# DCMMC/halo2-scaffold

Measured on AMD Instinct MI355X. Metric: create_proof() wall-clock + MSM G1-adds/s at k=20 standard_plonk, 1/2/4/8 GPU, higher is better.
Workload: dtype u32 (254-bit Montgomery integers as 9 x 29-bit limbs, 64-bit multiply-accumulate); 1 GPU; standard_plonk hot-path replay k=20: 11 MSM(2^20) + 6 iNTT(2^20) + 6 coset-NTT(2^21) + 1 coset-iNTT(2^21); k=20, scalar_distribution=uniform, msm_window_bits=17, msm_windows=15, msm_buckets=65536, parallelism=single-gpu, deployment=one process, one GPU, combine=none (single GPU)

## Files before the change

### halo2-scaffold_amd/csrc/f29.cuh

```cuda
#pragma once
#include <stdint.h>

#if defined(__HIPCC__)
#include <hip/hip_runtime.h>
#define H2_HD __host__ __device__ __forceinline__
#else
#define H2_HD inline
#endif

namespace h2 {

#include "f29_consts.inc"

constexpr uint32_t M29 = (1u << 29) - 1;

struct f29 {
  uint32_t v[9];
};

template <class F>
H2_HD f29 f29_const(const uint32_t (&c)[9]) {
  f29 r;
#pragma unroll
  for (int i = 0; i < 9; i++) r.v[i] = c[i];
  return r;
}
H2_HD f29 f29_zero() {
  f29 r;
#pragma unroll
  for (int i = 0; i < 9; i++) r.v[i] = 0;
  return r;
}
H2_HD bool f29_limbs_zero(const f29& a) {
  uint32_t o = 0;
#pragma unroll
  for (int i = 0; i < 9; i++) o |= a.v[i];
  return o == 0;
}

H2_HD f29 f29_unpack(const uint32_t w[8]) {
  f29 r;
#pragma unroll
  for (int i = 0; i < 9; i++) {
    const int bit = 29 * i, j = bit >> 5, s = bit & 31;
    uint32_t lo = w[j] >> s;
    if (s > 3 && j + 1 < 8) lo |= w[j + 1] << (32 - s);
    r.v[i] = (i < 8) ? (lo & M29) : lo;
  }
  return r;
}
H2_HD void f29_pack(const f29& a, uint32_t w[8]) {
#pragma unroll
  for (int j = 0; j < 8; j++) {
    const int bit = 32 * j, i = bit / 29, s = bit - 29 * i;
    uint32_t x = a.v[i] >> s;
    x |= a.v[i + 1] << (29 - s);
    if (29 - s + 29 < 32 && i + 2 < 9) x |= a.v[i + 2] << (58 - s);
    w[j] = x;
  }
}

H2_HD f29 f29_normalize(const f29& a) {
  f29 r;
  uint32_t c = 0;
#pragma unroll
  for (int i = 0; i < 8; i++) {
    uint32_t x = a.v[i] + c;
    r.v[i] = x & M29;
    c = x >> 29;
  }
  r.v[8] = a.v[8] + c;
  return r;
}

H2_HD f29 f29_add(const f29& a, const f29& b) {
  f29 r;
#pragma unroll
  for (int i = 0; i < 9; i++) r.v[i] = a.v[i] + b.v[i];
  return r;
}
H2_HD f29 f29_sub(const f29& a, const f29& b, const uint32_t (&K)[9]) {
  f29 r;
#pragma unroll
  for (int i = 0; i < 9; i++) r.v[i] = a.v[i] + K[i] - b.v[i];
  return r;
}
H2_HD f29 f29_dbl(const f29& a) {
  f29 r;
#pragma unroll
  for (int i = 0; i < 9; i++) r.v[i] = a.v[i] << 1;
  return r;
}

H2_HD void f29_mac_first(uint64_t& acc, uint32_t x, uint32_t y) {
#if defined(__HIP_DEVICE_COMPILE__)
  asm("v_mad_u64_u32 %0, vcc, %1, %2, %0" : "+v"(acc) : "v"(x), "v"(y) : "vcc");
#else
  acc += (uint64_t)x * y;
#endif
}

template <class F>
H2_HD f29 f29_mul(const f29& a, const f29& b) {
  uint32_t m[9];
  f29 t;
  uint64_t acc = 0;
#pragma unroll
  for (int k = 0; k < 9; k++) {
    f29_mac_first(acc, a.v[0], b.v[k]);
#pragma unroll
    for (int j = 1; j <= k; j++) acc += (uint64_t)a.v[j] * b.v[k - j];
#pragma unroll
    for (int j = 0; j < k; j++) acc += (uint64_t)m[j] * F::P[k - j];
    m[k] = ((uint32_t)acc * F::INV) & M29;
    acc += (uint64_t)m[k] * F::P[0];
    acc >>= 29;
  }
#pragma unroll
  for (int k = 9; k < 17; k++) {
    f29_mac_first(acc, a.v[k - 8], b.v[8]);
#pragma unroll
    for (int j = k - 7; j < 9; j++) acc += (uint64_t)a.v[j] * b.v[k - j];
#pragma unroll
    for (int j = k - 8; j < 9; j++) acc += (uint64_t)m[j] * F::P[k - j];
    t.v[k - 9] = (uint32_t)acc & M29;
    acc >>= 29;
  }
  t.v[8] = (uint32_t)acc;
  return t;
}
template <class F>
H2_HD f29 f29_mul2(const f29& a, const f29& b, const f29& c, const f29& d) {
  uint32_t m[9];
  f29 t;
  uint64_t acc = 0;
#pragma unroll
  for (int k = 0; k < 9; k++) {
    f29_mac_first(acc, a.v[0], b.v[k]);
#pragma unroll
    for (int j = 1; j <= k; j++) acc += (uint64_t)a.v[j] * b.v[k - j];
#pragma unroll
    for (int j = 0; j <= k; j++) acc += (uint64_t)c.v[j] * d.v[k - j];
#pragma unroll
    for (int j = 0; j < k; j++) acc += (uint64_t)m[j] * F::P[k - j];
    m[k] = ((uint32_t)acc * F::INV) & M29;
    acc += (uint64_t)m[k] * F::P[0];
    acc >>= 29;
  }
#pragma unroll
  for (int k = 9; k < 17; k++) {
    f29_mac_first(acc, a.v[k - 8], b.v[8]);
#pragma unroll
    for (int j = k - 7; j < 9; j++) acc += (uint64_t)a.v[j] * b.v[k - j];
#pragma unroll
    for (int j = k - 8; j < 9; j++) acc += (uint64_t)c.v[j] * d.v[k - j];
#pragma unroll
    for (int j = k - 8; j < 9; j++) acc += (uint64_t)m[j] * F::P[k - j];
    t.v[k - 9] = (uint32_t)acc & M29;
    acc >>= 29;
  }
  t.v[8] = (uint32_t)acc;
  return t;
}
template <class F>
H2_HD f29 f29_mul3(const f29& a, const f29& b, const f29& c, const f29& d, const f29& e, const f29& f) {
  uint32_t m[9];
  f29 t;
  uint64_t acc = 0;
#pragma unroll
  for (int k = 0; k < 9; k++) {
    f29_mac_first(acc, a.v[0], b.v[k]);
#pragma unroll
    for (int j = 1; j <= k; j++) acc += (uint64_t)a.v[j] * b.v[k - j];
#pragma unroll
    for (int j = 0; j <= k; j++) acc += (uint64_t)c.v[j] * d.v[k - j];
#pragma unroll
    for (int j = 0; j <= k; j++) acc += (uint64_t)e.v[j] * f.v[k - j];
#pragma unroll
    for (int j = 0; j < k; j++) acc += (uint64_t)m[j] * F::P[k - j];
    m[k] = ((uint32_t)acc * F::INV) & M29;
    acc += (uint64_t)m[k] * F::P[0];
    acc >>= 29;
  }
#pragma unroll
  for (int k = 9; k < 17; k++) {
    f29_mac_first(acc, a.v[k - 8], b.v[8]);
#pragma unroll
    for (int j = k - 7; j < 9; j++) acc += (uint64_t)a.v[j] * b.v[k - j];
#pragma unroll
    for (int j = k - 8; j < 9; j++) acc += (uint64_t)c.v[j] * d.v[k - j];
#pragma unroll
    for (int j = k - 8; j < 9; j++) acc += (uint64_t)e.v[j] * f.v[k - j];
#pragma unroll
    for (int j = k - 8; j < 9; j++) acc += (uint64_t)m[j] * F::P[k - j];
    t.v[k - 9] = (uint32_t)acc & M29;
    acc >>= 29;
  }
  t.v[8] = (uint32_t)acc;
  return t;
}
template <class F>
H2_HD f29 f29_sqr(const f29& a) {
  uint32_t m[9], a2[9];
#pragma unroll
  for (int i = 0; i < 9; i++) a2[i] = a.v[i] << 1;
  f29 t;
  uint64_t acc = 0;
#pragma unroll
  for (int k = 0; k < 9; k++) {
    if (k == 0) f29_mac_first(acc, a.v[0], a.v[0]);
    else f29_mac_first(acc, a.v[0], a2[k]);
#pragma unroll
    for (int j = 1; 2 * j < k; j++) acc += (uint64_t)a.v[j] * a2[k - j];
    if ((k & 1) == 0 && k > 0) acc += (uint64_t)a.v[k / 2] * a.v[k / 2];
#pragma unroll
    for (int j = 0; j < k; j++) acc += (uint64_t)m[j] * F::P[k - j];
    m[k] = ((uint32_t)acc * F::INV) & M29;
    acc += (uint64_t)m[k] * F::P[0];
    acc >>= 29;
  }
#pragma unroll
  for (int k = 9; k < 17; k++) {
    f29_mac_first(acc, m[k - 8], F::P[8]);
#pragma unroll
    for (int j = k - 8; 2 * j < k; j++) acc += (uint64_t)a.v[j] * a2[k - j];
    if ((k & 1) == 0) acc += (uint64_t)a.v[k / 2] * a.v[k / 2];
#pragma unroll
    for (int j = k - 7; j < 9; j++) acc += (uint64_t)m[j] * F::P[k - j];
    t.v[k - 9] = (uint32_t)acc & M29;
    acc >>= 29;
  }
  t.v[8] = (uint32_t)acc;
  return t;
}

template <class F>
H2_HD f29 f29_reduce_canonical(const f29& a) {
  f29 d;
  uint32_t borrow = 0;
#pragma unroll
  for (int i = 0; i < 9; i++) {
    uint32_t x = a.v[i] - F::P[i] - borrow;
    borrow = (x >> 31) & 1u;
    d.v[i] = (i < 8) ? (x & M29) : x;
  }
  f29 r;
#pragma unroll
  for (int i = 0; i < 9; i++) r.v[i] = borrow ? a.v[i] : d.v[i];
  return r;
}
template <class F>
H2_HD f29 f29_reduce_loose(const f29& a) {
  constexpr uint32_t M = (uint32_t)(((uint64_t)1 << 32) / (F::P[8] + 1));
  const uint32_t q = (uint32_t)(((uint64_t)a.v[8] * M) >> 32);
  f29 r;
  int64_t c = 0;
#pragma unroll
  for (int i = 0; i < 9; i++) {
    int64_t d = (int64_t)a.v[i] - (int64_t)((uint64_t)q * F::P[i]) + c;
    if (i < 8) {
      r.v[i] = (uint32_t)d & M29;
      c = d >> 29;
    } else {
      r.v[i] = (uint32_t)d;
    }
  }
  return f29_reduce_canonical<F>(f29_reduce_canonical<F>(r));
}

template <class F>
H2_HD bool f29_is_zero_mod(const f29& a) {
  if (a.v[0] != 0 && a.v[0] != F::P[0]) return false;
  uint32_t z = 0, e = 0;
#pragma unroll
  for (int i = 0; i < 9; i++) {
    z |= a.v[i];
    e |= a.v[i] ^ F::P[i];
  }
  return z == 0 || e == 0;
}

template <class F>
H2_HD f29 f29_inv(const f29& a) {
  f29 r = f29_const<F>(F::ONE);
  for (int i = 8; i >= 0; i--) {
    const uint32_t e = F::P[i] - (i == 0 ? 2u : 0u);
    const int top = (i == 8) ? 21 : 28;
    for (int b = top; b >= 0; b--) {
      r = f29_sqr<F>(r);
      if ((e >> b) & 1u) r = f29_mul<F>(r, a);
    }
  }
  return r;
}

template <class F>
H2_HD f29 f29_from_mont256(const uint32_t w[8]) {
  return f29_mul<F>(f29_unpack(w), f29_const<F>(F::TO261));
}
template <class F>
H2_HD void f29_to_mont256(const f29& a_norm, uint32_t w[8]) {
  f29 c = f29_reduce_canonical<F>(f29_mul<F>(a_norm, f29_const<F>(F::TO256)));
  f29_pack(c, w);
}

}
```

### halo2-scaffold_amd/csrc/f29_testops.cuh

```cuda
#pragma once
#include <stddef.h>

#include "g1_29.cuh"

namespace h2 {

template <class F>
H2_HD void f29t_mul_one(int mode, const uint32_t* a, const uint32_t* b, uint32_t* out) {
  if (mode == 0) {
    f29 x = f29_from_mont256<F>(a), y = f29_from_mont256<F>(b);
    f29_to_mont256<F>(f29_mul<F>(x, y), out);
  } else if (mode == 1) {
    f29 d = f29_unpack(a), w = f29_from_mont256<F>(b);
    f29 r = f29_reduce_canonical<F>(f29_mul<F>(d, w));
    f29_pack(r, out);
  } else if (mode == 2) {
    f29 x = f29_from_mont256<F>(a), y = f29_from_mont256<F>(b);
    f29 s = f29_normalize(f29_add(x, y));
    f29 d = f29_sub(x, y, F::K2);
    f29_to_mont256<F>(f29_mul<F>(d, s), out);
  } else if (mode == 4) {
    f29 x = f29_from_mont256<F>(a);
    f29_to_mont256<F>(f29_sqr<F>(x), out);
  } else if (mode == 5) {
    f29 x = f29_from_mont256<F>(a);
    f29_to_mont256<F>(f29_inv<F>(x), out);
  } else {
    f29 x = f29_unpack(a);
    f29_pack(x, out);
  }
}

H2_HD f29 f29t_load9(const uint32_t* p) {
  f29 x;
  for (int k = 0; k < 9; k++) x.v[k] = p[k];
  return x;
}
H2_HD void f29t_store9(const f29& x, uint32_t* p) {
  for (int k = 0; k < 9; k++) p[k] = x.v[k];
}

template <class F>
H2_HD void f29t_raw_one(int op, const uint32_t* a, const uint32_t* b, const uint32_t* c, const uint32_t* d, uint32_t* out) {
  f29 r;
  if (op == 0) r = f29_reduce_loose<F>(f29t_load9(a));
  else if (op == 1) r = f29_mul<F>(f29t_load9(a), f29t_load9(b));
  else if (op == 2) r = f29_sqr<F>(f29t_load9(a));
  else r = f29_mul2<F>(f29t_load9(a), f29t_load9(b), f29t_load9(c), f29t_load9(d));
  f29t_store9(r, out);
}
template <class F>
H2_HD void f29t_mul3_one(const uint32_t* ops, size_t n, size_t i, uint32_t* out) {
  f29 x[6];
  for (int q = 0; q < 6; q++) x[q] = f29t_load9(ops + ((size_t)q * n + i) * 9);
  f29t_store9(f29_mul3<F>(x[0], x[1], x[2], x[3], x[4], x[5]), out);
}

H2_HD bool f29t_table_point(const uint32_t* p, bool neg, f29& x2, f29& y2) {
  uint32_t any = 0;
  for (int k = 0; k < 16; k++) any |= p[k];
  if (any == 0) return false;
  uint32_t xw[8], yw[8];
  f29_pack(f29_reduce_canonical<Fq29>(f29_from_mont256<Fq29>(p)), xw);
  f29_pack(f29_reduce_canonical<Fq29>(f29_from_mont256<Fq29>(p + 8)), yw);
  x2 = f29_unpack(xw);
  y2 = f29_unpack(yw);
  if (neg) y2 = f29_sub(f29_zero(), y2, Fq29::K2);
  return true;
}

H2_HD void f29t_chain_one(const uint32_t* pts, const uint8_t* signs, size_t n, uint32_t* out_xyzz, int tree) {
  xyzz29 acc = xyzz29_identity();
  f29 x2, y2;
  if (!tree) {
    for (size_t i = 0; i < n; i++)
      if (f29t_table_point(pts + 16 * i, signs[i] != 0, x2, y2)) xyzz29_madd(acc, x2, y2);
  } else {
    xyzz29 groups[16];
    for (int g = 0; g < tree; g++) groups[g] = xyzz29_identity();
    for (size_t i = 0; i < n; i++)
      if (f29t_table_point(pts + 16 * i, signs[i] != 0, x2, y2)) xyzz29_madd(groups[i % tree], x2, y2);
    for (int stride = 1; stride < tree; stride *= 2)
      for (int g = 0; g + stride < tree; g += 2 * stride) xyzz29_add(groups[g], groups[g + stride]);
    acc = groups[0];
    if (tree == 16) {
      xyzz29 s2 = acc;
      xyzz29_add(s2, acc);
      xyzz29 d = xyzz29_dbl(acc);
      d.y = f29_normalize(f29_sub(f29_zero(), d.y, Fq29::K4));
      xyzz29_add(s2, d);
      xyzz29_add(s2, acc);
      acc = s2;
    }
  }
  if (xyzz29_is_identity(acc)) {
    for (int k = 0; k < 32; k++) out_xyzz[k] = 0;
    return;
  }
  f29_to_mont256<Fq29>(acc.x, out_xyzz);
  f29_to_mont256<Fq29>(acc.y, out_xyzz + 8);
  f29_to_mont256<Fq29>(acc.zz, out_xyzz + 16);
  f29_to_mont256<Fq29>(acc.zzz, out_xyzz + 24);
}

}
```

### halo2-scaffold_amd/csrc/g1_29.cuh

```cuda
#pragma once
#include "f29.cuh"

namespace h2 {

struct affine29 {
  f29 x, y;
};
struct xyzz29 {
  f29 x, y, zz, zzz;
};

H2_HD bool affine29_is_identity(const affine29& p) { return f29_limbs_zero(p.x) && f29_limbs_zero(p.y); }
H2_HD bool xyzz29_is_identity(const xyzz29& p) { return f29_limbs_zero(p.zz); }
H2_HD xyzz29 xyzz29_identity() {
  xyzz29 r;
  r.x = f29_zero(); r.y = f29_zero(); r.zz = f29_zero(); r.zzz = f29_zero();
  return r;
}

H2_HD xyzz29 xyzz29_dbl_affine(const f29& x, const f29& y_any) {
  using F = Fq29;
  xyzz29 r;
  f29 y = f29_normalize(y_any);
  f29 u = f29_normalize(f29_dbl(y));
  f29 v = f29_sqr<F>(u);
  f29 w = f29_mul<F>(u, v);
  f29 s = f29_mul<F>(x, v);
  f29 xx = f29_sqr<F>(x);
  f29 m = f29_normalize(f29_add(f29_dbl(xx), xx));
  f29 mm = f29_sqr<F>(m);
  r.x = f29_normalize(f29_sub(mm, f29_dbl(s), F::KW4));
  f29 t = f29_sub(s, r.x, F::K6);
  r.y = f29_mul2<F>(t, m, f29_sub(f29_zero(), y, F::K4), w);
  r.zz = v;
  r.zzz = w;
  return r;
}

H2_HD void xyzz29_madd(xyzz29& acc, const f29& x2, const f29& y2) {
  using F = Fq29;
  if (xyzz29_is_identity(acc)) {
    acc.x = x2;
    acc.y = f29_normalize(y2);
    acc.zz = f29_const<F>(F::ONE);
    acc.zzz = f29_const<F>(F::ONE);
    return;
  }
  f29 u2 = f29_mul<F>(x2, acc.zz);
  f29 s2 = f29_mul<F>(y2, acc.zzz);
  f29 p = f29_normalize(f29_sub(u2, acc.x, F::K6));
  f29 r = f29_normalize(f29_sub(s2, acc.y, F::K4));
  f29 pp = f29_sqr<F>(p);
  if (f29_is_zero_mod<F>(pp)) {
    f29 rr = f29_sqr<F>(r);
    if (f29_is_zero_mod<F>(rr)) acc = xyzz29_dbl_affine(x2, y2);
    else acc = xyzz29_identity();
    return;
  }
  f29 ppp = f29_mul<F>(p, pp);
  f29 q = f29_mul<F>(acc.x, pp);
  f29 rr = f29_sqr<F>(r);
  f29 sub3 = f29_add(ppp, f29_dbl(q));
  f29 x3 = f29_normalize(f29_sub(rr, sub3, F::KW4));
  f29 t = f29_sub(q, x3, F::K6);
  f29 ny = f29_sub(f29_zero(), acc.y, F::K4);
  acc.x = x3;
  acc.y = f29_mul2<F>(t, r, ny, ppp);
  acc.zz = f29_mul<F>(acc.zz, pp);
  acc.zzz = f29_mul<F>(acc.zzz, ppp);
}

H2_HD f29 affine29_pair_diff(const f29& x1, const f29& x2) { return f29_normalize(f29_sub(x2, x1, Fq29::K2)); }
H2_HD void affine29_pair_add(const f29& x1, const f29& y1, bool neg1, const f29& x2, const f29& y2, bool neg2, const f29& dinv, f29& x3, f29& y3) {
  using F = Fq29;
  f29 dy;
  if (neg1 == neg2) dy = neg2 ? f29_sub(y1, y2, F::K2) : f29_sub(y2, y1, F::K2);
  else dy = neg2 ? f29_sub(f29_zero(), f29_add(y1, y2), F::KW4) : f29_add(y1, y2);
  const f29 lam = f29_mul<F>(f29_normalize(dy), dinv);
  const f29 ll = f29_sqr<F>(lam);
  x3 = f29_normalize(f29_sub(ll, f29_add(x1, x2), F::KW4));
  const f29 t = f29_sub(x1, x3, F::K6);
  const f29 m = f29_mul<F>(t, lam);
  y3 = neg1 ? f29_add(m, y1) : f29_sub(m, y1, F::K2);
}

H2_HD xyzz29 xyzz29_dbl(const xyzz29& p) {
  using F = Fq29;
  if (xyzz29_is_identity(p)) return p;
  xyzz29 r;
  f29 u = f29_normalize(f29_dbl(p.y));
  f29 v = f29_sqr<F>(u);
  f29 w = f29_mul<F>(u, v);
  f29 s = f29_mul<F>(p.x, v);
  f29 xx = f29_sqr<F>(p.x);
  f29 m = f29_normalize(f29_add(f29_dbl(xx), xx));
  f29 mm = f29_sqr<F>(m);
  r.x = f29_normalize(f29_sub(mm, f29_dbl(s), F::KW4));
  f29 t = f29_sub(s, r.x, F::K6);
  r.y = f29_mul2<F>(t, m, f29_sub(f29_zero(), p.y, F::K4), w);
  r.zz = f29_mul<F>(v, p.zz);
  r.zzz = f29_mul<F>(w, p.zzz);
  return r;
}

H2_HD void xyzz29_add(xyzz29& a, const xyzz29& b) {
  using F = Fq29;
  if (xyzz29_is_identity(b)) return;
  if (xyzz29_is_identity(a)) { a = b; return; }
  f29 u1 = f29_mul<F>(a.x, b.zz);
  f29 u2 = f29_mul<F>(b.x, a.zz);
  f29 s1 = f29_mul<F>(a.y, b.zzz);
  f29 s2 = f29_mul<F>(b.y, a.zzz);
  f29 p = f29_normalize(f29_sub(u2, u1, F::K2));
  f29 r = f29_normalize(f29_sub(s2, s1, F::K2));
  f29 pp = f29_sqr<F>(p);
  if (f29_is_zero_mod<F>(pp)) {
    f29 rr0 = f29_sqr<F>(r);
    if (f29_is_zero_mod<F>(rr0)) a = xyzz29_dbl(a);
    else a = xyzz29_identity();
    return;
  }
  f29 ppp = f29_mul<F>(p, pp);
  f29 q = f29_mul<F>(u1, pp);
  f29 rr = f29_sqr<F>(r);
  f29 x3 = f29_normalize(f29_sub(rr, f29_add(ppp, f29_dbl(q)), F::KW4));
  f29 t = f29_sub(q, x3, F::K6);
  f29 zz = f29_mul<F>(f29_mul<F>(a.zz, b.zz), pp);
  f29 zzz = f29_mul<F>(f29_mul<F>(a.zzz, b.zzz), ppp);
  a.x = x3;
  a.y = f29_mul2<F>(t, r, f29_sub(f29_zero(), s1, F::K2), ppp);
  a.zz = zz;
  a.zzz = zzz;
}

H2_HD xyzz29 xyzz29_from_jacobian(const f29& x, const f29& y, const f29& z) {
  using F = Fq29;
  if (f29_limbs_zero(z)) return xyzz29_identity();
  xyzz29 r;
  r.x = x;
  r.y = y;
  r.zz = f29_sqr<F>(z);
  r.zzz = f29_mul<F>(r.zz, z);
  return r;
}
H2_HD void xyzz29_to_jacobian(const xyzz29& p, f29& x, f29& y, f29& z) {
  using F = Fq29;
  x = f29_mul<F>(p.x, p.zz);
  y = f29_mul<F>(p.y, p.zzz);
  z = p.zz;
}

H2_HD void xyzz29_to_affine(const xyzz29& p, f29& x, f29& y) {
  using F = Fq29;
  if (xyzz29_is_identity(p)) { x = f29_zero(); y = f29_zero(); return; }
  f29 zi = f29_inv<F>(p.zzz);
  y = f29_reduce_canonical<F>(f29_mul<F>(p.y, zi));
  f29 t = f29_mul<F>(p.zz, zi);
  x = f29_reduce_canonical<F>(f29_mul<F>(p.x, f29_sqr<F>(t)));
}

}
```

### halo2-scaffold_amd/csrc/h2mi_hooks.h

```cpp
#ifndef H2MI_HOOKS_H
#define H2MI_HOOKS_H
#include "../../include/h2mi.h"
#ifdef __cplusplus
extern "C" {
#endif
int h2mi_dbg_field_op(int field , int op ,
                      const uint64_t* a, const uint64_t* b, uint64_t* out, size_t n);
int h2mi_dbg_g1_op(int op, const uint64_t* p_affine, const uint64_t* q_affine, uint64_t* out_jac, size_t n);
int h2mi_dbg_g1_quad_op(int op, const uint64_t* p, const uint64_t* q_or_null, uint64_t* out_jac, size_t n);
int h2mi_dbg_f29_mul(int field, int mode, const uint32_t* a, const uint32_t* b, uint32_t* out, size_t n);
int h2mi_dbg_f29_reduce_loose(int field, const uint32_t* in9, uint32_t* out9, size_t n);
int h2mi_dbg_f29_mul_raw(int field, const uint32_t* a, const uint32_t* b, uint32_t* out, size_t n);
int h2mi_dbg_f29_sqr_raw(int field, const uint32_t* a, uint32_t* out, size_t n);
int h2mi_dbg_f29_mul2_raw(int field, const uint32_t* a, const uint32_t* b, const uint32_t* c, const uint32_t* d, uint32_t* out, size_t n);
int h2mi_dbg_f29_mul3_raw(int field, const uint32_t* ops , uint32_t* out, size_t n);
int h2mi_dbg_g1_29_chains(const uint32_t* pts, const uint8_t* signs, const uint64_t* offsets, size_t nchains, uint32_t* out_xyzz, int tree);
#ifdef __cplusplus
}
#endif
#endif
```

### halo2-scaffold_amd/csrc/h2mi_hooks.hip

```cpp
#include "g1.cuh"
#include "f29_testops.cuh"
#include "g1_29_quad.cuh"
#include "h2mi_hooks.h"
#include "h2mi_internal.h"

namespace h2 {

template <class F>
__global__ void __launch_bounds__(256) k_dbg_field(int op, const fe* a, const fe* b, fe* out, size_t n) {
  size_t i = (size_t)blockIdx.x * blockDim.x + threadIdx.x;
  if (i >= n) return;
  fe x = fe_load(&a[i]);
  fe y = b ? fe_load(&b[i]) : fe_zero();
  fe r;
  switch (op) {
    case 0: r = fe_mul<F>(x, y); break;
    case 1: r = fe_add<F>(x, y); break;
    case 2: r = fe_sub<F>(x, y); break;
    case 3: r = fe_sqr<F>(x); break;
    case 5: r = fe_from_mont<F>(x); break;
    case 6: r = fe_to_mont<F>(x); break;
    case 7: r = fe_neg<F>(x); break;
    case 9: r = fe_inv_ds<F>(x); break;
    case 10: r = fe_inv_gcd<F>(x); break;
// ... 51 lines not shown
  size_t i = (size_t)blockIdx.x * blockDim.x + threadIdx.x;
  if (i >= n) return;
  f29t_raw_one<F>(op, a + 9 * i, b ? b + 9 * i : nullptr, c ? c + 9 * i : nullptr, d ? d + 9 * i : nullptr, out + 9 * i);
}
template <class F>
__global__ void __launch_bounds__(256) k_dbg_f29_mul3(const uint32_t* ops, uint32_t* out, size_t n) {
  size_t i = (size_t)blockIdx.x * blockDim.x + threadIdx.x;
  if (i >= n) return;
  f29t_mul3_one<F>(ops, n, i, out + 9 * i);
}
__global__ void __launch_bounds__(64) k_dbg_g1_29_chains(const uint32_t* pts, const uint8_t* signs, const uint64_t* offsets, size_t nchains, uint32_t* out, int tree) {
  size_t c = (size_t)blockIdx.x * blockDim.x + threadIdx.x;
  if (c >= nchains) return;
  const uint64_t lo = offsets[c], hi = offsets[c + 1];
  f29t_chain_one(pts + 16 * lo, signs + lo, (size_t)(hi - lo), out + 32 * c, tree);
}

}

using namespace h2;

template <class Launch>
static int f29_dbg_run(const uint32_t* const* ops, int nops, size_t words, size_t owords, uint32_t* out, size_t n, Launch launch) {
  std::lock_guard<std::recursive_mutex> lk(ctx().mu);
  hipStream_t s = ctx().stream;
  DevMem d[4], dout;
  for (int q = 0; q < nops; q++) {
    if (!ops[q]) continue;
    H2_HIP(d[q].alloc(n * words * 4));
    H2_HIP(hipMemcpyAsync(d[q].p, ops[q], n * words * 4, hipMemcpyHostToDevice, s));
  }
  H2_HIP(dout.alloc(n * owords * 4));
  int rc = launch(s, d, dout.as<uint32_t>());
  if (rc) return rc;
  H2_HIP(hipMemcpyAsync(out, dout.p, n * owords * 4, hipMemcpyDeviceToHost, s));
  H2_HIP(hipStreamSynchronize(s));
  return H2MI_OK;
}

static int f29_dbg_raw(int field, int op, const uint32_t* a, const uint32_t* b, const uint32_t* c, const uint32_t* d, uint32_t* out, size_t n) {
  const uint32_t* ops[4] = {a, b, c, d};
  return f29_dbg_run(ops, 4, 9, 9, out, n, [&](hipStream_t s, DevMem* m, uint32_t* dout) {
    const uint32_t grid = ceil_div_u32(n, 256);
    if (field == 0) {
      H2_LAUNCH("k_dbg_f29_raw_fq", k_dbg_f29_raw<Fq29>, grid, 256, 0, s, op, m[0].as<uint32_t>(), m[1].as<uint32_t>(), m[2].as<uint32_t>(), m[3].as<uint32_t>(), dout, n);
    } else {
      H2_LAUNCH("k_dbg_f29_raw_fr", k_dbg_f29_raw<Fr29>, grid, 256, 0, s, op, m[0].as<uint32_t>(), m[1].as<uint32_t>(), m[2].as<uint32_t>(), m[3].as<uint32_t>(), dout, n);
    }
    return (int)H2MI_OK;
  });
}

extern "C" {

int h2mi_dbg_field_op(int field, int op, const uint64_t* a, const uint64_t* b, uint64_t* out, size_t n) {
  H2_REQUIRE_INIT();
  if (!a || !out || n == 0 || op < 0 || op > 10 || op == 4) return H2MI_EINVAL;
  std::lock_guard<std::recursive_mutex> lk(ctx().mu);
  hipStream_t s = ctx().stream;
  DevMem da, db, dout;
  H2_HIP(da.alloc(n * 32));
  H2_HIP(dout.alloc(n * 32));
  H2_HIP(hipMemcpyAsync(da.p, a, n * 32, hipMemcpyHostToDevice, s));
  if (b) {
    H2_HIP(db.alloc(n * 32));
    H2_HIP(hipMemcpyAsync(db.p, b, n * 32, hipMemcpyHostToDevice, s));
  }
  uint32_t grid = ceil_div_u32(n, 256);
  if (field == 0) {
    H2_LAUNCH("k_dbg_field_fq", k_dbg_field<FqP>, grid, 256, 0, s, op, da.as<fe>(), db.as<fe>(), dout.as<fe>(), n);
  } else {
    H2_LAUNCH("k_dbg_field_fr", k_dbg_field<FrP>, grid, 256, 0, s, op, da.as<fe>(), db.as<fe>(), dout.as<fe>(), n);
  }
  H2_HIP(hipMemcpyAsync(out, dout.p, n * 32, hipMemcpyDeviceToHost, s));
  H2_HIP(hipStreamSynchronize(s));
  return H2MI_OK;
}


int h2mi_dbg_g1_op(int op, const uint64_t* p, const uint64_t* q, uint64_t* out_jac, size_t n) {
  H2_REQUIRE_INIT();
  if (!p || !out_jac || n == 0 || (op != 1 && !q)) return H2MI_EINVAL;
  std::lock_guard<std::recursive_mutex> lk(ctx().mu);
  hipStream_t s = ctx().stream;
  DevMem dp, dq, dout;
  H2_HIP(dp.alloc(n * 64));
  H2_HIP(dout.alloc(n * 96));
  H2_HIP(hipMemcpyAsync(dp.p, p, n * 64, hipMemcpyHostToDevice, s));
  if (q) {
    H2_HIP(dq.alloc(n * 64));
    H2_HIP(hipMemcpyAsync(dq.p, q, n * 64, hipMemcpyHostToDevice, s));
  }
  H2_LAUNCH("k_dbg_g1", k_dbg_g1, ceil_div_u32(n, 256), 256, 0, s, op, dp.as<uint8_t>(), dq.as<uint8_t>(), dout.as<uint8_t>(), n);
  H2_HIP(hipMemcpyAsync(out_jac, dout.p, n * 96, hipMemcpyDeviceToHost, s));
  H2_HIP(hipStreamSynchronize(s));
  return H2MI_OK;
}


int h2mi_dbg_g1_quad_op(int op, const uint64_t* p, const uint64_t* q, uint64_t* out_jac, size_t n) {
  H2_REQUIRE_INIT();
  if (!p || !out_jac || n == 0 || (op != 0 && op != 1) || (op == 0 && !q)) return H2MI_EINVAL;
  std::lock_guard<std::recursive_mutex> lk(ctx().mu);
  hipStream_t s = ctx().stream;
  DevMem dp, dq, dout;
  H2_HIP(dp.alloc(n * 64));
  H2_HIP(dout.alloc(n * 96));
  H2_HIP(hipMemcpyAsync(dp.p, p, n * 64, hipMemcpyHostToDevice, s));
  if (q) {
    H2_HIP(dq.alloc(n * 64));
    H2_HIP(hipMemcpyAsync(dq.p, q, n * 64, hipMemcpyHostToDevice, s));
  }
  H2_LAUNCH("k_dbg_quad", k_dbg_quad, ceil_div_u32(n * 4, 256), 256, 0, s, op, dp.as<uint8_t>(), dq.as<uint8_t>(), dout.as<uint8_t>(), n);
  H2_HIP(hipMemcpyAsync(out_jac, dout.p, n * 96, hipMemcpyDeviceToHost, s));
  H2_HIP(hipStreamSynchronize(s));
  return H2MI_OK;
}

int h2mi_dbg_f29_mul(int field, int mode, const uint32_t* a, const uint32_t* b, uint32_t* out, size_t n) {
  H2_REQUIRE_INIT();
  if (!a || !b || !out || n == 0 || (field != 0 && field != 1) || mode < 0 || mode > 5) return H2MI_EINVAL;
  const uint32_t* ops[2] = {a, b};
  return f29_dbg_run(ops, 2, 8, 8, out, n, [&](hipStream_t s, DevMem* m, uint32_t* dout) {
    const uint32_t grid = ceil_div_u32(n, 256);
    if (field == 0) {
      H2_LAUNCH("k_dbg_f29_mul_fq", k_dbg_f29_mul<Fq29>, grid, 256, 0, s, mode, m[0].as<uint32_t>(), m[1].as<uint32_t>(), dout, n);
    } else {
      H2_LAUNCH("k_dbg_f29_mul_fr", k_dbg_f29_mul<Fr29>, grid, 256, 0, s, mode, m[0].as<uint32_t>(), m[1].as<uint32_t>(), dout, n);
    }
    return (int)H2MI_OK;
  });
}

int h2mi_dbg_f29_reduce_loose(int field, const uint32_t* in9, uint32_t* out9, size_t n) {
  H2_REQUIRE_INIT();
  if (!in9 || !out9 || n == 0 || (field != 0 && field != 1)) return H2MI_EINVAL;
  return f29_dbg_raw(field, 0, in9, nullptr, nullptr, nullptr, out9, n);
}
int h2mi_dbg_f29_mul_raw(int field, const uint32_t* a, const uint32_t* b, uint32_t* out, size_t n) {
  H2_REQUIRE_INIT();
  if (!a || !b || !out || n == 0 || (field != 0 && field != 1)) return H2MI_EINVAL;
  return f29_dbg_raw(field, 1, a, b, nullptr, nullptr, out, n);
}
int h2mi_dbg_f29_sqr_raw(int field, const uint32_t* a, uint32_t* out, size_t n) {
  H2_REQUIRE_INIT();
  if (!a || !out || n == 0 || (field != 0 && field != 1)) return H2MI_EINVAL;
  return f29_dbg_raw(field, 2, a, nullptr, nullptr, nullptr, out, n);
}
int h2mi_dbg_f29_mul2_raw(int field, const uint32_t* a, const uint32_t* b, const uint32_t* c, const uint32_t* d, uint32_t* out, size_t n) {
  H2_REQUIRE_INIT();
  if (!a || !b || !c || !d || !out || n == 0 || (field != 0 && field != 1)) return H2MI_EINVAL;
  return f29_dbg_raw(field, 3, a, b, c, d, out, n);
}
int h2mi_dbg_f29_mul3_raw(int field, const uint32_t* ops, uint32_t* out, size_t n) {
  H2_REQUIRE_INIT();
  if (!ops || !out || n == 0 || (field != 0 && field != 1)) return H2MI_EINVAL;
  const uint32_t* one[1] = {ops};
  return f29_dbg_run(one, 1, 6 * 9, 9, out, n, [&](hipStream_t s, DevMem* m, uint32_t* dout) {
    const uint32_t grid = ceil_div_u32(n, 256);
    if (field == 0) {
      H2_LAUNCH("k_dbg_f29_mul3_fq", k_dbg_f29_mul3<Fq29>, grid, 256, 0, s, m[0].as<uint32_t>(), dout, n);
    } else {
      H2_LAUNCH("k_dbg_f29_mul3_fr", k_dbg_f29_mul3<Fr29>, grid, 256, 0, s, m[0].as<uint32_t>(), dout, n);
    }
    return (int)H2MI_OK;
  });
}

int h2mi_dbg_g1_29_chains(const uint32_t* pts, const uint8_t* signs, const uint64_t* offsets, size_t nchains, uint32_t* out_xyzz, int tree) {
  H2_REQUIRE_INIT();
  if (!pts || !signs || !offsets || !out_xyzz || nchains == 0) return H2MI_EINVAL;
  if (tree != 0 && tree != 2 && tree != 4 && tree != 8 && tree != 16) return H2MI_EINVAL;
  if (offsets[0] != 0) return H2MI_EINVAL;
  for (size_t c = 0; c < nchains; c++)
    if (offsets[c + 1] < offsets[c]) return H2MI_EINVAL;
  const size_t npts = offsets[nchains];
  std::lock_guard<std::recursive_mutex> lk(ctx().mu);
  hipStream_t s = ctx().stream;
  DevMem dp, ds, doff, dout;
  H2_HIP(dp.alloc(npts * 64));
  H2_HIP(ds.alloc(npts));
  H2_HIP(doff.alloc((nchains + 1) * 8));
  H2_HIP(dout.alloc(nchains * 128));
  H2_HIP(hipMemcpyAsync(dp.p, pts, npts * 64, hipMemcpyHostToDevice, s));
  H2_HIP(hipMemcpyAsync(ds.p, signs, npts, hipMemcpyHostToDevice, s));
  H2_HIP(hipMemcpyAsync(doff.p, offsets, (nchains + 1) * 8, hipMemcpyHostToDevice, s));
  H2_LAUNCH("k_dbg_g1_29_chains", k_dbg_g1_29_chains, ceil_div_u32(nchains, 64), 64, 0, s, dp.as<uint32_t>(), ds.as<uint8_t>(), doff.as<uint64_t>(), nchains,
            dout.as<uint32_t>(), tree);
  H2_HIP(hipMemcpyAsync(out_xyzz, dout.p, nchains * 128, hipMemcpyDeviceToHost, s));
  H2_HIP(hipStreamSynchronize(s));
  return H2MI_OK;
}

}
```

### halo2-scaffold_amd/csrc/h2mi_msm.hip

```cpp

#include <algorithm>
#include <map>
#include <type_traits>
#include <vector>

#include "g1.cuh"
#include "g1_29.cuh"
#include "g1_29_quad.cuh"
#include "h2mi_internal.h"
#include "scan.cuh"

namespace h2 {

constexpr uint32_t S0_MAX = 128;
constexpr uint32_t S1 = 8;
constexpr uint32_t FG_NARROW = 8;
constexpr uint32_t FG_WIDE = 2;
constexpr size_t SHIFT_MIN_N = 4096;
constexpr uint32_t HOT_MIN = 64;
constexpr uint32_t HOT_MIN_WIDE = 8;

constexpr uint32_t ACCUM_RESIDENT_CHUNKS = 256 * 2 * 256;
__host__ __device__ inline uint32_t accum_rounds(uint32_t entries) {
  const uint32_t per_round = S0_MAX * ACCUM_RESIDENT_CHUNKS;
// ... 451 lines not shown
    __syncthreads();
    for (uint32_t p = tid; p < m; p += P2_THREADS) {
      const uint32_t qq = stage_q[p];
      vals_out[run[qq] + (p - cstart[qq])] = stage[p];
    }
    __syncthreads();
    if (tid < NQ_MAX) {
      run[tid] += ccnt[tid];
      ccnt[tid] = 0;
    }
    __syncthreads();
  }
}
__global__ void __launch_bounds__(P2_THREADS) k_msm_bin_sort(const uint8_t* keys_in, const uint32_t* vals_in, const uint32_t* base, uint32_t ntiles,
                                                             uint32_t nbins, uint32_t lb, uint32_t s0_fixed, uint32_t nb, uint32_t* vals_out,
                                                             uint32_t* off, uint32_t* np0, uint32_t* np1, uint32_t* s0_out) {
  msm_bin_sort_body(keys_in, vals_in, base, ntiles, nbins, lb, s0_fixed, nb, vals_out, off, np0, np1, s0_out);
}

constexpr uint32_t NQW = 1024, P2W_PER = 12, P2W_CH = P2_THREADS * P2W_PER;
__device__ __forceinline__ void block_excl_scan_1024(const uint32_t* in, uint32_t* out, uint32_t* wtot ) {
  const uint32_t tid = threadIdx.x, lane = tid & 63, wave = tid >> 6;
  const uint32_t a = in[2 * tid], b = in[2 * tid + 1];
  const uint32_t inc = wave_incl_scan(a + b);
  if (lane == 63) wtot[wave] = inc;
  __syncthreads();
  uint32_t add = 0;
  for (uint32_t w = 0; w < wave; w++) add += wtot[w];
  const uint32_t ex = add + inc - (a + b);
  __syncthreads();
  out[2 * tid] = ex;
  out[2 * tid + 1] = ex + a;
}
__global__ void __launch_bounds__(P2_THREADS) k_msm_bin_sort_wide(const uint16_t* keys_in, const uint32_t* vals_in, const uint32_t* base,
                                                                  uint32_t ntiles, uint32_t nbins, uint32_t lb, uint32_t s0_fixed, uint32_t nb,
                                                                  uint32_t* vals_out, uint32_t* off, uint32_t* np0, uint32_t* np1, uint32_t* s0_out) {
  __shared__ uint32_t hist[NQW], run[NQW], ccnt[NQW], cstart[NQW], wtot[P2_THREADS / 64];
  __shared__ uint32_t stage[P2W_CH];
  __shared__ uint16_t stage_q[P2W_CH];
  const uint32_t tid = threadIdx.x, bin = blockIdx.x;
  const uint32_t start = base[(size_t)bin * ntiles], end = base[(size_t)(bin + 1) * ntiles];
  const uint32_t nq = 1u << lb;
  const uint32_t entries = base[(size_t)nbins * ntiles];
  const uint32_t s0 = s0_fixed ? s0_fixed : accum_chunk_len(entries);
  for (uint32_t j = tid; j < NQW; j += P2_THREADS) {
    hist[j] = 0;
    ccnt[j] = 0;
  }
  __syncthreads();
  for (uint32_t j = (start & ~7u) + tid * 8; j < end; j += P2_THREADS * 8) {
    const uint4 kk = *reinterpret_cast<const uint4*>(keys_in + j);
    const uint32_t w4[4] = {kk.x, kk.y, kk.z, kk.w};
#pragma unroll
    for (uint32_t t = 0; t < 8; t++) {
      const uint32_t idx = j + t;
      if (idx >= start && idx < end) atomicAdd(&hist[(w4[t >> 1] >> (16 * (t & 1))) & (NQW - 1)], 1u);
    }
  }
  __syncthreads();
  block_excl_scan_1024(hist, cstart, wtot);
  __syncthreads();
  for (uint32_t q = tid; q < NQW; q += P2_THREADS) {
    const uint32_t ex = cstart[q], tot = hist[q];
    run[q] = start + ex;
    if (q < nq) {
      const uint32_t b = (bin << lb) + q;
      const uint32_t o = start + ex;
      off[b] = o;
      const uint32_t f0 = tot ? 1u + (o + tot - 1) / s0 - o / s0 : 0u;
      np0[b] = f0;
      np1[b] = (f0 + S1 - 1) / S1;
    }
  }
  if (bin == 0 && tid == 0) {
    off[nb] = entries;
    np0[nb] = 0;
    np1[nb] = 0;
    *s0_out = s0;
  }
  __syncthreads();
  for (uint32_t cs = start; cs < end; cs += P2W_CH) {
    const uint32_t m = min(P2W_CH, end - cs);
    uint32_t q[P2W_PER], v[P2W_PER], r[P2W_PER];
#pragma unroll
    for (uint32_t k = 0; k < P2W_PER; k++) {
      const uint32_t p = k * P2_THREADS + tid;
      if (p < m) {
        q[k] = keys_in[cs + p] & (NQW - 1);
        v[k] = vals_in[cs + p];
      }
    }
#pragma unroll
    for (uint32_t k = 0; k < P2W_PER; k++)
      if (k * P2_THREADS + tid < m) r[k] = atomicAdd(&ccnt[q[k]], 1u);
    __syncthreads();
    block_excl_scan_1024(ccnt, cstart, wtot);
    __syncthreads();
#pragma unroll
    for (uint32_t k = 0; k < P2W_PER; k++)
      if (k * P2_THREADS + tid < m) {
        const uint32_t pos = cstart[q[k]] + r[k];
        stage[pos] = v[k];
        stage_q[pos] = (uint16_t)q[k];
      }
    __syncthreads();
    for (uint32_t p = tid; p < m; p += P2_THREADS) {
      const uint32_t qq = stage_q[p];
      vals_out[run[qq] + (p - cstart[qq])] = stage[p];
    }
    __syncthreads();
    for (uint32_t qi = tid; qi < NQW; qi += P2_THREADS) {
      run[qi] += ccnt[qi];
      ccnt[qi] = 0;
    }
    __syncthreads();
  }
}

constexpr uint32_t PART_BYTES = 144;
__device__ __forceinline__ xyzz29 part_load(const uint8_t* p) {
  const uint4* q = reinterpret_cast<const uint4*>(p);
  uint32_t w[36];
#pragma unroll
  for (int i = 0; i < 9; i++) {
    uint4 v = q[i];
    w[4 * i] = v.x; w[4 * i + 1] = v.y; w[4 * i + 2] = v.z; w[4 * i + 3] = v.w;
  }
  xyzz29 r;
#pragma unroll
  for (int i = 0; i < 9; i++) { r.x.v[i] = w[i]; r.y.v[i] = w[9 + i]; r.zz.v[i] = w[18 + i]; r.zzz.v[i] = w[27 + i]; }
  return r;
}
__device__ __forceinline__ void part_store(uint8_t* p, const xyzz29& a) {
  uint32_t w[36];
#pragma unroll
  for (int i = 0; i < 9; i++) { w[i] = a.x.v[i]; w[9 + i] = a.y.v[i]; w[18 + i] = a.zz.v[i]; w[27 + i] = a.zzz.v[i]; }
  uint4* q = reinterpret_cast<uint4*>(p);
#pragma unroll
  for (int i = 0; i < 9; i++) q[i] = make_uint4(w[4 * i], w[4 * i + 1], w[4 * i + 2], w[4 * i + 3]);
}

__device__ __forceinline__ uint32_t find_bucket(const uint32_t* toff, uint32_t nb, uint32_t t) {
  uint32_t lo = 0, hi = nb;
  while (hi - lo > 1) {
    uint32_t mid = (lo + hi) >> 1;
    if (toff[mid] <= t) lo = mid;
    else hi = mid;
  }
  return lo;
}

typedef affine tab_entry;
__device__ __forceinline__ tab_entry tab_load(const uint8_t* table, uint32_t i) { return affine_load(table + (size_t)i * 64); }
__device__ __forceinline__ bool tab_is_identity(const tab_entry& p) { return affine_is_identity(p); }
__device__ __forceinline__ f29 tab_x(const tab_entry& p) { return f29_unpack(p.x.v); }
__device__ __forceinline__ f29 tab_y(const tab_entry& p) { return f29_unpack(p.y.v); }

__device__ __forceinline__ void msm_accum_body(const uint32_t* entries, const uint32_t* off, const uint32_t* toff, uint32_t nb, const uint32_t* s0_dev,
                                               const uint8_t* table, uint8_t* part) {
  const uint32_t t = blockIdx.x * blockDim.x + threadIdx.x;
  const uint32_t total = off[nb];
  const uint32_t s0 = *s0_dev;
  if ((uint64_t)t * s0 >= total) return;
  const uint32_t start = t * s0;
  const uint32_t end = min(start + s0, total);
  uint32_t b = find_bucket(off, nb, start);
  uint32_t pidx = toff[b] + (t - off[b] / s0);
  uint32_t bend = off[b + 1];
  xyzz29 acc = xyzz29_identity();
  uint32_t e = entries[start];
  tab_entry nxt = tab_load(table, e & 0x7fffffffu);
  uint32_t nneg = e >> 31;
  for (uint32_t k = start; k < end; k++) {
    if (k == bend) {
      part_store(part + (size_t)pidx * PART_BYTES, acc);
      pidx++;
      acc = xyzz29_identity();
      do {
        b++;
        bend = off[b + 1];
      } while (bend == k);
    }
    tab_entry p = nxt;
    uint32_t neg = nneg;
    if (k + 1 < end) {
      e = entries[k + 1];
      nxt = tab_load(table, e & 0x7fffffffu);
      nneg = e >> 31;
    }
    if (tab_is_identity(p)) continue;
    f29 x2 = tab_x(p);
    f29 y2 = tab_y(p);
    if (neg) y2 = f29_sub(f29_zero(), y2, Fq29::K2);
    xyzz29_madd(acc, x2, y2);
  }
  part_store(part + (size_t)pidx * PART_BYTES, acc);
}
__global__ void __launch_bounds__(256) k_msm_accum(const uint32_t* entries, const uint32_t* off, const uint32_t* toff, uint32_t nb,
                                                    const uint32_t* s0_dev, const uint8_t* table, uint8_t* part) {
  msm_accum_body(entries, off, toff, nb, s0_dev, table, part);
}

constexpr size_t ACCUM_LDS = 56000;

constexpr uint32_t HEAD_BATCH = 4;
struct HeadDesc {
  const fe* scalars;
  fe* shift;
  uint32_t *bincnt, *tile_live, *binseg, *binbase, *vals0, *vals1, *off, *np0, *np1, *toff0, *toff1, *s0_dev;
  void* bkeys;
  uint8_t* part0;
};
struct HeadBatch {
  HeadDesc d[HEAD_BATCH];
};
__global__ void __launch_bounds__(64) k_msm_pick_shift_b(const HeadBatch hb, size_t n) {
  const HeadDesc& d = hb.d[blockIdx.y];
  msm_pick_shift_body(d.scalars, n, d.shift);
}
template <uint32_t CT>
__global__ void __launch_bounds__(P1_TS) k_msm_bin_count_b(const HeadBatch hb, size_t n, uint32_t c, uint32_t W, uint32_t lb, uint32_t nbins,
                                                           uint32_t ntiles) {
  const HeadDesc& d = hb.d[blockIdx.y];
  msm_bin_count_body<CT>(d.scalars, n, d.shift, c, W, lb, nbins, ntiles, d.bincnt, d.tile_live);
}
template <uint32_t CT>
__global__ void __launch_bounds__(P1_TS) k_msm_bin_scatter_b(const HeadBatch hb, size_t n, size_t n_reg, uint32_t c, uint32_t W, uint32_t lb,
                                                             uint32_t nbins, uint32_t ntiles) {
  const HeadDesc& d = hb.d[blockIdx.y];
  msm_bin_scatter_body<CT>(d.scalars, n, d.shift, n_reg, c, W, lb, nbins, ntiles, d.binbase, d.vals0, d.bkeys, d.tile_live);
}
__global__ void __launch_bounds__(P2_THREADS) k_msm_bin_sort_b(const HeadBatch hb, uint32_t ntiles, uint32_t nbins, uint32_t lb, uint32_t s0_fixed,
                                                               uint32_t nb) {
  const HeadDesc& d = hb.d[blockIdx.y];
  msm_bin_sort_body((const uint8_t*)d.bkeys, d.vals0, d.binbase, ntiles, nbins, lb, s0_fixed, nb, d.vals1, d.off, d.np0, d.np1, d.s0_dev);
}
__global__ void __launch_bounds__(256) k_msm_accum_b(const HeadBatch hb, uint32_t nb, const uint8_t* table) {
  const HeadDesc& d = hb.d[blockIdx.y];
  msm_accum_body(d.vals1, d.off, d.toff0, nb, d.s0_dev, table, d.part0);
}
__global__ void __launch_bounds__(1024) k_scan_segsum_bins_b(const HeadBatch hb, uint32_t m) {
  const HeadDesc& d = hb.d[blockIdx.y];
  scan_segsum_body<SCAN_SEG_BINS>(d.bincnt, m, d.binseg);
}
__global__ void __launch_bounds__(1024) k_scan_seg_bins_b(const HeadBatch hb, uint32_t m) {
  const HeadDesc& d = hb.d[blockIdx.y];
  scan_seg_body<SCAN_SEG_BINS>(d.bincnt, d.binbase, m, d.binseg);
}
__global__ void __launch_bounds__(1024) k_scan_seg_tasks_b(const HeadBatch hb, uint32_t m) {
  const HeadDesc& d = hb.d[blockIdx.z];
  scan_seg_body<SCAN_SEG_TASKS>(blockIdx.y ? d.np1 : d.np0, blockIdx.y ? d.toff1 : d.toff0, m, nullptr);
}

constexpr uint32_t TAIL_BATCH = 8;
struct TailDesc {
  const uint8_t* part0;
  const uint32_t *toff0, *np0, *toff1, *np1, *off;
  uint8_t *part1, *dense, *rc, *g, *out;
  uint64_t* stats;
  uint32_t nb, logNh, logNl, canonical;
  const uint8_t* mat;
  uint8_t *dense2, *vsum;
  uint32_t seg_log;
  uint32_t hot_min;
  uint32_t no_fold;
};
struct TailBatch {
  TailDesc d[TAIL_BATCH];
};

constexpr uint32_t TAIL_THREADS = 512;

template <bool QUAD>
__global__ void __launch_bounds__(256) k_msm_fold(const TailBatch tb) {
  const TailDesc& d = tb.d[blockIdx.y];
  if (d.no_fold) return;
  const uint32_t nb = d.nb;
  const uint32_t *toff_out = d.toff1, *toff_in = d.toff0, *np_in = d.np0;
  const uint32_t t = (blockIdx.x * blockDim.x + threadIdx.x) >> (QUAD ? 2 : 0);
  if (t >= toff_out[nb]) return;
  uint32_t b = find_bucket(toff_out, nb, t);
  uint32_t j = t - toff_out[b];
  const uint32_t m = np_in[b], np = toff_out[b + 1] - toff_out[b];
  const uint32_t q = m / np, r = m - q * np;
  uint32_t start = toff_in[b] + j * q + min(j, r);
  uint32_t len = q + (j < r ? 1u : 0u);
  xyzz29 acc = part_load(d.part0 + (size_t)start * PART_BYTES);
  for (uint32_t k = 1; k < len; k++) {
    xyzz29 p = part_load(d.part0 + (size_t)(start + k) * PART_BYTES);
    if (QUAD) acc = xyzz29_add_quad(acc, p);
    else xyzz29_add(acc, p);
  }
  if (!QUAD || (threadIdx.x & 3u) == 0) part_store(d.part1 + (size_t)t * PART_BYTES, acc);
}

__device__ __forceinline__ xyzz29 shfl_down_xyzz(const xyzz29& a, uint32_t delta) {
  xyzz29 r;
#pragma unroll
  for (int i = 0; i < 9; i++) {
    r.x.v[i] = __shfl_down(a.x.v[i], delta);
    r.y.v[i] = __shfl_down(a.y.v[i], delta);
    r.zz.v[i] = __shfl_down(a.zz.v[i], delta);
    r.zzz.v[i] = __shfl_down(a.zzz.v[i], delta);
  }
  return r;
}
__device__ __forceinline__ void msm_finish_hot_body(const TailDesc& d, uint32_t bx);
template <bool QUAD, uint32_t FG>
__global__ void __launch_bounds__(256) k_msm_finish(const TailBatch tb, uint32_t hot_blocks) {
  const TailDesc& d = tb.d[blockIdx.y];
  if (blockIdx.x < hot_blocks) {
    msm_finish_hot_body(d, blockIdx.x);
    return;
  }
  const uint32_t bx = blockIdx.x - hot_blocks;
  const uint32_t nb = d.nb;
  constexpr uint32_t LW = QUAD ? 2 : 0;
  const uint32_t worker = (bx * blockDim.x + threadIdx.x) >> LW;
  const uint32_t b = worker / FG, l = worker % FG;
  if ((bx * blockDim.x >> LW) / FG >= nb) return;
  xyzz29 acc = xyzz29_identity();
  bool hot = false;
  if (b < nb) {
    uint32_t cnt = d.np1[b], s = d.toff1[b];
    hot = cnt > d.hot_min;
    if (hot) cnt = 0;
    for (uint32_t k = l; k < cnt; k += FG) {
      xyzz29 p = part_load(d.part1 + (size_t)(s + k) * PART_BYTES);
      if (QUAD) acc = xyzz29_add_quad(acc, p);
      else xyzz29_add(acc, p);
    }
  }
  for (uint32_t dd = FG / 2; dd > 0; dd >>= 1) {
    xyzz29 o = shfl_down_xyzz(acc, dd << LW);
    if (l < dd) {
      if (QUAD) acc = xyzz29_add_quad(acc, o);
      else xyzz29_add(acc, o);
    }
  }
  if (b < nb && !hot && l == 0 && (!QUAD || (threadIdx.x & 3u) == 0)) part_store(d.dense + (size_t)b * PART_BYTES, acc);
}

__device__ __forceinline__ void block_tree_sum(xyzz29* lds, uint32_t count_pow2) {
  const uint32_t quad = threadIdx.x >> 2, nquads = blockDim.x >> 2;
  for (uint32_t s = count_pow2 >> 1; s > 0; s >>= 1) {
    for (uint32_t g = quad; g < s; g += nquads) {
// ... 1338 lines not shown
```

Before: 9.795 billion G1-adds/s.

## Fuse Montgomery add into mul/sqr and restructure MSM accumulate prefetch

Adds fused multiply-add and square-add variants that fold an addend into the final carry chain of the Montgomery product. EC doubling and addition formulas use them to drop separate normalize and sub passes. The MSM accumulate loop also reorders its prefetch: it unpacks the current point before loading the next one, and clamps the index instead of branching. This cuts register pressure and ALU work in the hot bucket-accumulate path, but the fused addend may exceed the limb bounds the old separate normalization guaranteed.

```diff
diff --git a/halo2-scaffold_amd/csrc/f29.cuh b/halo2-scaffold_amd/csrc/f29.cuh
--- a/halo2-scaffold_amd/csrc/f29.cuh
+++ b/halo2-scaffold_amd/csrc/f29.cuh
@@ -100,8 +100,8 @@
 #endif
 }
 
-template <class F>
-H2_HD f29 f29_mul(const f29& a, const f29& b) {
+template <class F, bool ADD>
+H2_HD f29 f29_mul_impl(const f29& a, const f29& b, const f29* c) {
   uint32_t m[9];
   f29 t;
   uint64_t acc = 0;
@@ -123,11 +123,21 @@
     for (int j = k - 7; j < 9; j++) acc += (uint64_t)a.v[j] * b.v[k - j];
 #pragma unroll
     for (int j = k - 8; j < 9; j++) acc += (uint64_t)m[j] * F::P[k - j];
+    if constexpr (ADD) f29_mac_first(acc, c->v[k - 9], 1u);
     t.v[k - 9] = (uint32_t)acc & M29;
     acc >>= 29;
   }
   t.v[8] = (uint32_t)acc;
+  if constexpr (ADD) t.v[8] += c->v[8];
   return t;
+}
+template <class F>
+H2_HD f29 f29_mul(const f29& a, const f29& b) {
+  return f29_mul_impl<F, false>(a, b, nullptr);
+}
+template <class F>
+H2_HD f29 f29_mul_add(const f29& a, const f29& b, const f29& c) {
+  return f29_mul_impl<F, true>(a, b, &c);
 }
 template <class F>
 H2_HD f29 f29_mul2(const f29& a, const f29& b, const f29& c, const f29& d) {
@@ -199,8 +209,8 @@
   t.v[8] = (uint32_t)acc;
   return t;
 }
-template <class F>
-H2_HD f29 f29_sqr(const f29& a) {
+template <class F, bool ADD>
+H2_HD f29 f29_sqr_impl(const f29& a, const f29* c) {
   uint32_t m[9], a2[9];
 #pragma unroll
   for (int i = 0; i < 9; i++) a2[i] = a.v[i] << 1;
@@ -227,11 +237,21 @@
     if ((k & 1) == 0) acc += (uint64_t)a.v[k / 2] * a.v[k / 2];
 #pragma unroll
     for (int j = k - 7; j < 9; j++) acc += (uint64_t)m[j] * F::P[k - j];
+    if constexpr (ADD) f29_mac_first(acc, c->v[k - 9], 1u);
     t.v[k - 9] = (uint32_t)acc & M29;
     acc >>= 29;
   }
   t.v[8] = (uint32_t)acc;
+  if constexpr (ADD) t.v[8] += c->v[8];
   return t;
+}
+template <class F>
+H2_HD f29 f29_sqr(const f29& a) {
+  return f29_sqr_impl<F, false>(a, nullptr);
+}
+template <class F>
+H2_HD f29 f29_sqr_add(const f29& a, const f29& c) {
+  return f29_sqr_impl<F, true>(a, &c);
 }
 
 template <class F>
diff --git a/halo2-scaffold_amd/csrc/f29_testops.cuh b/halo2-scaffold_amd/csrc/f29_testops.cuh
--- a/halo2-scaffold_amd/csrc/f29_testops.cuh
+++ b/halo2-scaffold_amd/csrc/f29_testops.cuh
@@ -46,6 +46,10 @@
   if (op == 0) r = f29_reduce_loose<F>(f29t_load9(a));
   else if (op == 1) r = f29_mul<F>(f29t_load9(a), f29t_load9(b));
   else if (op == 2) r = f29_sqr<F>(f29t_load9(a));
+  else if (op == 4) r = f29_mul_add<F>(f29t_load9(a), f29t_load9(b), f29t_load9(c));
+  else if (op == 5) r = f29_normalize(f29_add(f29_mul<F>(f29t_load9(a), f29t_load9(b)), f29t_load9(c)));
+  else if (op == 6) r = f29_sqr_add<F>(f29t_load9(a), f29t_load9(c));
+  else if (op == 7) r = f29_normalize(f29_add(f29_sqr<F>(f29t_load9(a)), f29t_load9(c)));
   else r = f29_mul2<F>(f29t_load9(a), f29t_load9(b), f29t_load9(c), f29t_load9(d));
   f29t_store9(r, out);
 }
diff --git a/halo2-scaffold_amd/csrc/g1_29.cuh b/halo2-scaffold_amd/csrc/g1_29.cuh
--- a/halo2-scaffold_amd/csrc/g1_29.cuh
+++ b/halo2-scaffold_amd/csrc/g1_29.cuh
@@ -28,8 +28,7 @@
   f29 s = f29_mul<F>(x, v);
   f29 xx = f29_sqr<F>(x);
   f29 m = f29_normalize(f29_add(f29_dbl(xx), xx));
-  f29 mm = f29_sqr<F>(m);
-  r.x = f29_normalize(f29_sub(mm, f29_dbl(s), F::KW4));
+  r.x = f29_sqr_add<F>(m, f29_sub(f29_zero(), f29_dbl(s), F::KW4));
   f29 t = f29_sub(s, r.x, F::K6);
   r.y = f29_mul2<F>(t, m, f29_sub(f29_zero(), y, F::K4), w);
   r.zz = v;
@@ -46,10 +45,9 @@
     acc.zzz = f29_const<F>(F::ONE);
     return;
   }
-  f29 u2 = f29_mul<F>(x2, acc.zz);
-  f29 s2 = f29_mul<F>(y2, acc.zzz);
-  f29 p = f29_normalize(f29_sub(u2, acc.x, F::K6));
-  f29 r = f29_normalize(f29_sub(s2, acc.y, F::K4));
+  f29 ny = f29_sub(f29_zero(), acc.y, F::K4);
+  f29 p = f29_mul_add<F>(x2, acc.zz, f29_sub(f29_zero(), acc.x, F::K6));
+  f29 r = f29_mul_add<F>(y2, acc.zzz, ny);
   f29 pp = f29_sqr<F>(p);
   if (f29_is_zero_mod<F>(pp)) {
     f29 rr = f29_sqr<F>(r);
@@ -59,11 +57,9 @@
   }
   f29 ppp = f29_mul<F>(p, pp);
   f29 q = f29_mul<F>(acc.x, pp);
-  f29 rr = f29_sqr<F>(r);
   f29 sub3 = f29_add(ppp, f29_dbl(q));
-  f29 x3 = f29_normalize(f29_sub(rr, sub3, F::KW4));
+  f29 x3 = f29_sqr_add<F>(r, f29_sub(f29_zero(), sub3, F::KW4));
   f29 t = f29_sub(q, x3, F::K6);
-  f29 ny = f29_sub(f29_zero(), acc.y, F::K4);
   acc.x = x3;
   acc.y = f29_mul2<F>(t, r, ny, ppp);
   acc.zz = f29_mul<F>(acc.zz, pp);
@@ -94,8 +90,7 @@
   f29 s = f29_mul<F>(p.x, v);
   f29 xx = f29_sqr<F>(p.x);
   f29 m = f29_normalize(f29_add(f29_dbl(xx), xx));
-  f29 mm = f29_sqr<F>(m);
-  r.x = f29_normalize(f29_sub(mm, f29_dbl(s), F::KW4));
+  r.x = f29_sqr_add<F>(m, f29_sub(f29_zero(), f29_dbl(s), F::KW4));
   f29 t = f29_sub(s, r.x, F::K6);
   r.y = f29_mul2<F>(t, m, f29_sub(f29_zero(), p.y, F::K4), w);
   r.zz = f29_mul<F>(v, p.zz);
@@ -108,11 +103,10 @@
   if (xyzz29_is_identity(b)) return;
   if (xyzz29_is_identity(a)) { a = b; return; }
   f29 u1 = f29_mul<F>(a.x, b.zz);
-  f29 u2 = f29_mul<F>(b.x, a.zz);
   f29 s1 = f29_mul<F>(a.y, b.zzz);
-  f29 s2 = f29_mul<F>(b.y, a.zzz);
-  f29 p = f29_normalize(f29_sub(u2, u1, F::K2));
-  f29 r = f29_normalize(f29_sub(s2, s1, F::K2));
+  f29 ns1 = f29_sub(f29_zero(), s1, F::K2);
+  f29 p = f29_mul_add<F>(b.x, a.zz, f29_sub(f29_zero(), u1, F::K2));
+  f29 r = f29_mul_add<F>(b.y, a.zzz, ns1);
   f29 pp = f29_sqr<F>(p);
   if (f29_is_zero_mod<F>(pp)) {
     f29 rr0 = f29_sqr<F>(r);
@@ -122,13 +116,12 @@
   }
   f29 ppp = f29_mul<F>(p, pp);
   f29 q = f29_mul<F>(u1, pp);
-  f29 rr = f29_sqr<F>(r);
-  f29 x3 = f29_normalize(f29_sub(rr, f29_add(ppp, f29_dbl(q)), F::KW4));
+  f29 x3 = f29_sqr_add<F>(r, f29_sub(f29_zero(), f29_add(ppp, f29_dbl(q)), F::KW4));
   f29 t = f29_sub(q, x3, F::K6);
   f29 zz = f29_mul<F>(f29_mul<F>(a.zz, b.zz), pp);
   f29 zzz = f29_mul<F>(f29_mul<F>(a.zzz, b.zzz), ppp);
   a.x = x3;
-  a.y = f29_mul2<F>(t, r, f29_sub(f29_zero(), s1, F::K2), ppp);
+  a.y = f29_mul2<F>(t, r, ns1, ppp);
   a.zz = zz;
   a.zzz = zzz;
 }
diff --git a/halo2-scaffold_amd/csrc/h2mi_hooks.h b/halo2-scaffold_amd/csrc/h2mi_hooks.h
--- a/halo2-scaffold_amd/csrc/h2mi_hooks.h
+++ b/halo2-scaffold_amd/csrc/h2mi_hooks.h
@@ -14,6 +14,8 @@
 int h2mi_dbg_f29_sqr_raw(int field, const uint32_t* a, uint32_t* out, size_t n);
 int h2mi_dbg_f29_mul2_raw(int field, const uint32_t* a, const uint32_t* b, const uint32_t* c, const uint32_t* d, uint32_t* out, size_t n);
 int h2mi_dbg_f29_mul3_raw(int field, const uint32_t* ops , uint32_t* out, size_t n);
+int h2mi_dbg_f29_mul_add_raw(int field, int fused, const uint32_t* a, const uint32_t* b, const uint32_t* c, uint32_t* out, size_t n);
+int h2mi_dbg_f29_sqr_add_raw(int field, int fused, const uint32_t* a, const uint32_t* c, uint32_t* out, size_t n);
 int h2mi_dbg_g1_29_chains(const uint32_t* pts, const uint8_t* signs, const uint64_t* offsets, size_t nchains, uint32_t* out_xyzz, int tree);
 #ifdef __cplusplus
 }
diff --git a/halo2-scaffold_amd/csrc/h2mi_hooks.hip b/halo2-scaffold_amd/csrc/h2mi_hooks.hip
--- a/halo2-scaffold_amd/csrc/h2mi_hooks.hip
+++ b/halo2-scaffold_amd/csrc/h2mi_hooks.hip
@@ -227,6 +227,16 @@
   if (!a || !b || !c || !d || !out || n == 0 || (field != 0 && field != 1)) return H2MI_EINVAL;
   return f29_dbg_raw(field, 3, a, b, c, d, out, n);
 }
+int h2mi_dbg_f29_mul_add_raw(int field, int fused, const uint32_t* a, const uint32_t* b, const uint32_t* c, uint32_t* out, size_t n) {
+  H2_REQUIRE_INIT();
+  if (!a || !b || !c || !out || n == 0 || (field != 0 && field != 1)) return H2MI_EINVAL;
+  return f29_dbg_raw(field, fused ? 4 : 5, a, b, c, nullptr, out, n);
+}
+int h2mi_dbg_f29_sqr_add_raw(int field, int fused, const uint32_t* a, const uint32_t* c, uint32_t* out, size_t n) {
+  H2_REQUIRE_INIT();
+  if (!a || !c || !out || n == 0 || (field != 0 && field != 1)) return H2MI_EINVAL;
+  return f29_dbg_raw(field, fused ? 6 : 7, a, nullptr, c, nullptr, out, n);
+}
 int h2mi_dbg_f29_mul3_raw(int field, const uint32_t* ops, uint32_t* out, size_t n) {
   H2_REQUIRE_INIT();
   if (!ops || !out || n == 0 || (field != 0 && field != 1)) return H2MI_EINVAL;
diff --git a/halo2-scaffold_amd/csrc/h2mi_msm.hip b/halo2-scaffold_amd/csrc/h2mi_msm.hip
--- a/halo2-scaffold_amd/csrc/h2mi_msm.hip
+++ b/halo2-scaffold_amd/csrc/h2mi_msm.hip
@@ -627,7 +627,6 @@
 
 typedef affine tab_entry;
 __device__ __forceinline__ tab_entry tab_load(const uint8_t* table, uint32_t i) { return affine_load(table + (size_t)i * 64); }
-__device__ __forceinline__ bool tab_is_identity(const tab_entry& p) { return affine_is_identity(p); }
 __device__ __forceinline__ f29 tab_x(const tab_entry& p) { return f29_unpack(p.x.v); }
 __device__ __forceinline__ f29 tab_y(const tab_entry& p) { return f29_unpack(p.y.v); }
 
@@ -644,8 +643,8 @@
   uint32_t bend = off[b + 1];
   xyzz29 acc = xyzz29_identity();
   uint32_t e = entries[start];
-  tab_entry nxt = tab_load(table, e & 0x7fffffffu);
-  uint32_t nneg = e >> 31;
+  tab_entry p = tab_load(table, e & 0x7fffffffu);
+  uint32_t neg = e >> 31;
   for (uint32_t k = start; k < end; k++) {
     if (k == bend) {
       part_store(part + (size_t)pidx * PART_BYTES, acc);
@@ -656,17 +655,14 @@
         bend = off[b + 1];
       } while (bend == k);
     }
-    tab_entry p = nxt;
-    uint32_t neg = nneg;
-    if (k + 1 < end) {
-      e = entries[k + 1];
-      nxt = tab_load(table, e & 0x7fffffffu);
-      nneg = e >> 31;
-    }
-    if (tab_is_identity(p)) continue;
-    f29 x2 = tab_x(p);
+    const f29 x2 = tab_x(p);
     f29 y2 = tab_y(p);
+    const bool skip = f29_limbs_zero(x2) && f29_limbs_zero(y2);
     if (neg) y2 = f29_sub(f29_zero(), y2, Fq29::K2);
+    e = entries[min(k + 1, end - 1)];
+    p = tab_load(table, e & 0x7fffffffu);
+    neg = e >> 31;
+    if (skip) continue;
     xyzz29_madd(acc, x2, y2);
   }
   part_store(part + (size_t)pidx * PART_BYTES, acc);
```

After: 9.723 billion G1-adds/s. About the same (-0.7%).
